# Z2PackDev/TBmodels

Measured on AMD Instinct MI355X. Metric: k-points/sec (H(k)+eig) at N_orb=64, N_R=4096, higher is better.
Workload: dtype f64; 1 GPU; cfg2: dense N_orb=64 N_R=4096, 100000 random k-points per GPU, eigenval (H(k)+eig); kpoints_per_gpu=100000, collective=none, rccl_ranks=0, eigensolver=auto

## Files before the change

### tbmodels_amd/csrc/tbk_eig_small.hip

```cpp

#include <cstdlib>
#include <type_traits>

#include "tbk_dpp.h"
#include "tbk_internal.h"

namespace {

typedef double d2 __attribute__((ext_vector_type(2)));

template <int CTRL>
__device__ __forceinline__ double dpp_mov(double v) {
    int lo = __double2loint(v), hi = __double2hiint(v);
    lo = __builtin_amdgcn_update_dpp(0, lo, CTRL, 0xf, 0xf, true);
    hi = __builtin_amdgcn_update_dpp(0, hi, CTRL, 0xf, 0xf, true);
    return __hiloint2double(hi, lo);
}

__device__ __forceinline__ double wave_sum(double v) {
    v += dpp_mov<0x128>(v);
    v += dpp_mov<0x124>(v);
    v += dpp_mov<0x122>(v);
    v += dpp_mov<0x121>(v);
    {
        const unsigned lo = (unsigned)__double2loint(v), hi = (unsigned)__double2hiint(v);
        const auto rl = __builtin_amdgcn_permlane16_swap(lo, lo, false, false);
        const auto rh = __builtin_amdgcn_permlane16_swap(hi, hi, false, false);
        v = __hiloint2double((int)rh[0], (int)rl[0]) + __hiloint2double((int)rh[1], (int)rl[1]);
    }
    {
        const unsigned lo = (unsigned)__double2loint(v), hi = (unsigned)__double2hiint(v);
        const auto rl = __builtin_amdgcn_permlane32_swap(lo, lo, false, false);
        const auto rh = __builtin_amdgcn_permlane32_swap(hi, hi, false, false);
        v = __hiloint2double((int)rh[0], (int)rl[0]) + __hiloint2double((int)rh[1], (int)rl[1]);
    }
    return v;
}

__device__ __forceinline__ void wg_sync() {
    asm volatile("s_waitcnt lgkmcnt(0)" ::: "memory");
    __syncthreads();
}

__device__ __forceinline__ double bcast(double v, int lane) { return __shfl(v, lane, 64); }
__device__ __forceinline__ double bcast_uniform(double v, int lane) {
    const int lo = __builtin_amdgcn_readlane(__double2loint(v), lane);
    const int hi = __builtin_amdgcn_readlane(__double2hiint(v), lane);
    return __hiloint2double(hi, lo);
}

__device__ __forceinline__ double fast_rcp(double x) {
    double r = __builtin_amdgcn_rcp(x);
    double e = fma(-x, r, 1.0);
    r = fma(r, e, r);
    e = fma(-x, r, 1.0);
    return fma(r, e, r);
}
__device__ __forceinline__ void fast_sqrt_rsqrt(double x, double& root, double& rroot) {
    double r = __builtin_amdgcn_rsq(x);
    double g = x * r, h = 0.5 * r;
    double e = fma(-h, g, 0.5);
    g = fma(g, e, g);
    h = fma(h, e, h);
    e = fma(-h, g, 0.5);
    g = fma(g, e, g);
    h = fma(h, e, h);
    const double d = fma(-g, g, x);
    root = fma(d, h, g);
    rroot = 2.0 * h;
    e = fma(-root, rroot, 1.0);
    rroot = fma(rroot, e, rroot);
}


__device__ __forceinline__ void wave_lds_fence() { asm volatile("s_waitcnt lgkmcnt(0)" ::: "memory"); }

template <int SEG>
__device__ __forceinline__ double seg_sum(double v) {
    if (SEG == 8) {
        v += dpp_mov<0x141>(v);
        v += dpp_mov<0xB1>(v);
        v += dpp_mov<0x4E>(v);
        return v;
    }
    v += dpp_mov<0x128>(v);
    v += dpp_mov<0x124>(v);
    v += dpp_mov<0x122>(v);
    v += dpp_mov<0x121>(v);
    if (SEG == 32) {
        const unsigned lo = (unsigned)__double2loint(v), hi = (unsigned)__double2hiint(v);
        const auto rl = __builtin_amdgcn_permlane16_swap(lo, lo, false, false);
        const auto rh = __builtin_amdgcn_permlane16_swap(hi, hi, false, false);
        v = __hiloint2double((int)rh[0], (int)rl[0]) + __hiloint2double((int)rh[1], (int)rl[1]);
    }
    return v;
}

template <int NRP>
__global__ void __launch_bounds__(64)
herm_tridiag_packed_kernel(const double* __restrict__ H, int n, int64_t nk, double* __restrict__ D,
                           double* __restrict__ E, int64_t h_stride, int ldd, int off) {
    constexpr int G = 64 / NRP;
    constexpr int CG = 4;
    constexpr int NGR = NRP / CG;
    __shared__ d2 sv[64];
    __shared__ d2 sw[64];
    const int lane = threadIdx.x;
    const int row = lane % NRP;
    const int base = lane - row;
    const int64_t mat = (int64_t)blockIdx.x * G + lane / NRP;
    const bool live = mat < nk;
    const int64_t mc = live ? mat : nk - 1;
    const double* Hm = H + (size_t)mc * h_stride;
    double* Dm = D + (size_t)mc * ldd + off;
    double* Em = E + (size_t)mc * ldd + off;

    double ar[NRP], ai[NRP];
    {
        constexpr int LB = NRP <= 16 ? NRP : 16;
        const int li = min(row, n - 1);
        static_for<0, NRP / LB>([&](auto hc) {
            constexpr int c0 = decltype(hc)::value * LB;
            d2 raw[LB];
#pragma unroll
            for (int u = 0; u < LB; ++u) {
                const int cc = min(c0 + u, n - 1);
                const int lo = min(li, cc), hi = max(li, cc);
                raw[u] = *reinterpret_cast<const d2*>(Hm + ((size_t)lo * n + hi) * 2);
            }
#pragma unroll
            for (int u = 0; u < LB; ++u) {
                const int c = c0 + u;
                const bool inside = row < n && c < n;
                ar[c] = inside ? raw[u][0] : 0.0;
                ai[c] = inside ? (c >= row ? raw[u][1] : -raw[u][1]) : 0.0;
            }
        });
    }
    double xr = ar[0], xi = ai[0];

    constexpr bool BC = NRP >= 16;
    constexpr int NB = NRP >= 16 ? NRP / 16 : 1;
    auto spread = [&](double x, double (&o)[NB]) {
        if constexpr (NRP == 32) {
            const unsigned xl = (unsigned)__double2loint(x), xh = (unsigned)__double2hiint(x);
            const auto rl = __builtin_amdgcn_permlane16_swap(xl, xl, false, false);
            const auto rh = __builtin_amdgcn_permlane16_swap(xh, xh, false, false);
            o[0] = __hiloint2double((int)rh[0], (int)rl[0]);
            o[NB - 1] = __hiloint2double((int)rh[1], (int)rl[1]);
        } else {
            o[0] = x;
        }
    };

    for (int j = 0; j < n - 1; ++j) {
        if (live && row == j) Dm[j] = xr;
        const double alr = __shfl(xr, base + j + 1, 64), ali = __shfl(xi, base + j + 1, 64);
        const bool below = (row > j + 1) && (row < n);
        const double sigma = seg_sum<NRP>(below ? (xr * xr + xi * xi) : 0.0);
        const bool done = (sigma == 0.0) && (ali == 0.0);
        double root, rroot;
        fast_sqrt_rsqrt(done ? 1.0 : alr * alr + ali * ali + sigma, root, rroot);
        const double beta = done ? alr : -copysign(root, alr);
        const double rbeta = done ? 0.0 : -copysign(rroot, alr);
        const double tr = (beta - alr) * rbeta, ti = -ali * rbeta;
        const double qr = alr - beta, qi = ali;
        const double qn = done ? 0.0 : fast_rcp(qr * qr + qi * qi);
        const double scr = qr * qn, sci = -qi * qn;
        if (live && row == 0) Em[j] = beta;

        double vr = 0.0, vi = 0.0;
        if (below) {
            vr = xr * scr - xi * sci;
            vi = xr * sci + xi * scr;
        } else if (row == j + 1) {
            vr = 1.0;
        }
        double vbr[NB], vbi[NB];
        if constexpr (BC) {
            spread(vr, vbr);
            spread(vi, vbi);
        } else {
            wave_lds_fence();
            sv[lane] = (d2){vr, vi};
            wave_lds_fence();
        }

        double pr = 0.0, pi = 0.0;
        {
            double par[CG], pai[CG];
#pragma unroll
            for (int cc = 0; cc < CG; ++cc) par[cc] = pai[cc] = 0.0;
            static_for<0, NGR>([&](auto grc) {
                constexpr int gr = decltype(grc)::value;
                if (gr * CG + CG - 1 > j) {
                    if constexpr (BC) {
                        static_for<0, CG>([&](auto ccc) {
                            constexpr int cc = decltype(ccc)::value, c = gr * CG + cc;
                            fmac_bc<c & 15>(par[cc], vbr[c >> 4], ar[c]);
                            fmac_bc<c & 15>(pai[cc], vbi[c >> 4], ar[c]);
                            fnmac_bc<c & 15>(par[cc], vbi[c >> 4], ai[c]);
                            fmac_bc<c & 15>(pai[cc], vbr[c >> 4], ai[c]);
                        });
                    } else {
                        d2 vb[CG];
#pragma unroll
                        for (int cc = 0; cc < CG; ++cc) vb[cc] = sv[base + gr * CG + cc];
#pragma unroll
                        for (int cc = 0; cc < CG; ++cc) {
                            par[cc] = fma(ar[gr * CG + cc], vb[cc][0], par[cc]);
                            pai[cc] = fma(ar[gr * CG + cc], vb[cc][1], pai[cc]);
                        }
#pragma unroll
                        for (int cc = 0; cc < CG; ++cc) {
                            par[cc] = fma(-ai[gr * CG + cc], vb[cc][1], par[cc]);
                            pai[cc] = fma(ai[gr * CG + cc], vb[cc][0], pai[cc]);
                        }
                    }
                }
            });
#pragma unroll
            for (int cc = 0; cc < CG; ++cc) {
                pr += par[cc];
                pi += pai[cc];
            }
        }
        if (!((row > j) && (row < n))) pr = pi = 0.0;
        const double rho = seg_sum<NRP>(pr * vr + pi * vi);
        const double a2 = -0.5 * (tr * tr + ti * ti) * rho;
        const double wr = fma(a2, vr, pr * tr - pi * ti);
        const double wi = fma(a2, vi, pr * ti + pi * tr);
        double wbr[NB], wbi[NB];
        if constexpr (BC) {
            spread(wr, wbr);
            spread(wi, wbi);
        } else {
            sw[lane] = (d2){wr, wi};
            wave_lds_fence();
        }

        double nxr = 0.0, nxi = 0.0;
        static_for<0, NGR>([&](auto grc) {
            constexpr int gr = decltype(grc)::value;
            if (gr * CG + CG - 1 > j) {
                if constexpr (BC) {
                    static_for<0, CG>([&](auto ccc) {
                        constexpr int cc = decltype(ccc)::value, c = gr * CG + cc;
                        double r = ar[c], mm = ai[c];
                        fnmac_bc<c & 15>(r, wbr[c >> 4], vr);
                        fnmac_bc<c & 15>(mm, wbr[c >> 4], vi);
                        fnmac_bc<c & 15>(r, wbi[c >> 4], vi);
                        fmac_bc<c & 15>(mm, wbi[c >> 4], vr);
                        fnmac_bc<c & 15>(r, vbr[c >> 4], wr);
                        fnmac_bc<c & 15>(mm, vbr[c >> 4], wi);
                        fnmac_bc<c & 15>(r, vbi[c >> 4], wi);
                        fmac_bc<c & 15>(mm, vbi[c >> 4], wr);
                        ar[c] = r;
                        ai[c] = mm;
                        if (c == j + 1) {
                            nxr = r;
                            nxi = mm;
                        }
                    });
                } else {
                    d2 vb[CG], wb[CG];
#pragma unroll
                    for (int cc = 0; cc < CG; ++cc) {
                        vb[cc] = sv[base + gr * CG + cc];
                        wb[cc] = sw[base + gr * CG + cc];
                    }
#pragma unroll
                    for (int cc = 0; cc < CG; ++cc) {
                        const int c = gr * CG + cc;
                        ar[c] = fma(-vr, wb[cc][0], ar[c]);
                        ai[c] = fma(-vi, wb[cc][0], ai[c]);
                        ar[c] = fma(-vi, wb[cc][1], ar[c]);
                        ai[c] = fma(vr, wb[cc][1], ai[c]);
                        ar[c] = fma(-wr, vb[cc][0], ar[c]);
                        ai[c] = fma(-wi, vb[cc][0], ai[c]);
                        ar[c] = fma(-wi, vb[cc][1], ar[c]);
                        ai[c] = fma(wr, vb[cc][1], ai[c]);
                        if (c == j + 1) {
                            nxr = ar[c];
                            nxi = ai[c];
                        }
                    }
                }
            }
        });
        xr = nxr;
        xi = nxi;
    }
    if (live && row == n - 1) Dm[n - 1] = xr;
    if (live && row == 0) Em[n - 1] = 0.0;
}

struct HhScalars {
    d2 tau;
    d2 flag;
};

template <int NR, int NW>
__global__ void __launch_bounds__(NW * 64, NW == 2 ? 2 : 4)
herm_tridiag4_kernel(double* H, int n, double* __restrict__ D, double* __restrict__ E, int n_steps, int64_t h_stride, int ldd,
                     int off) {
    const bool split = n_steps < n - 1;
    constexpr int NT = NR / NW;
    constexpr int NB = (NT + 15) / 16;
    constexpr int TB = 2;
    constexpr int HT = NT / NB;
    static_assert(NT % NB == 0, "columns per lane must split evenly over the register arrays");
    typedef double dcol __attribute__((ext_vector_type(HT)));
    __shared__ d2 sx[2][NR];
    __shared__ HhScalars ssc;
    __shared__ d2 sp[NW][NR];
    __shared__ d2 sw[NR];
    const int lane = threadIdx.x & 63;
    const int q = __builtin_amdgcn_readfirstlane(threadIdx.x >> 6);
    const size_t mat = blockIdx.x;
    double* Hm = H + mat * (size_t)h_stride;
    double* Dm = D + mat * (size_t)ldd + off;
    double* Em = E + mat * (size_t)ldd + off;

    dcol ar0, ai0, ar1, ai1;
    static_assert(NB <= 2, "at most 32 columns per lane");
    auto AR = [&](auto bc) -> dcol& { if constexpr (decltype(bc)::value == 0) return ar0; else return ar1; };
    auto AI = [&](auto bc) -> dcol& { if constexpr (decltype(bc)::value == 0) return ai0; else return ai1; };
#define TBK_AR(t) AR(std::integral_constant<int, (t) / HT>{})[(t) % HT]
#define TBK_AI(t) AI(std::integral_constant<int, (t) / HT>{})[(t) % HT]
    {
        constexpr int LB = NT <= 16 ? NT : NT / 2;
        const int li = min(lane, n - 1);
        static_for<0, NT / LB>([&](auto t0c) {
            constexpr int t0 = decltype(t0c)::value * LB;
            d2 raw[LB];
#pragma unroll
            for (int u = 0; u < LB; ++u) {
                const int c = min(NW * (t0 + u) + q, n - 1);
                const int lo = min(li, c), hi = max(li, c);
                raw[u] = *reinterpret_cast<const d2*>(Hm + ((size_t)lo * n + hi) * 2);
            }
            static_for<0, LB>([&](auto uc) {
                constexpr int u = decltype(uc)::value;
                const int c = NW * (t0 + u) + q;
                const bool inside = lane < n && c < n;
                TBK_AR(t0 + u) = inside ? raw[u][0] : 0.0;
                TBK_AI(t0 + u) = inside ? (c >= lane ? raw[u][1] : -raw[u][1]) : 0.0;
            });
        });
    }

    auto publish = [&](int jc) {
        const int tsel = jc / NW;
        double xr, xi;
        if (NB == 1 || tsel < HT) {
            xr = ar0[tsel % HT];
            xi = ai0[tsel % HT];
        } else {
            xr = ar1[tsel % HT];
            xi = ai1[tsel % HT];
        }
        if (lane == jc) Dm[jc] = xr;
        if (jc >= n - 1) {
            if (lane == 0) Em[n - 1] = 0.0;
            return;
        }
        const double alr = bcast_uniform(xr, jc + 1), ali = bcast_uniform(xi, jc + 1);
        const bool below = (lane > jc + 1) && (lane < n);
        const double sigma = wave_sum(below ? (xr * xr + xi * xi) : 0.0);
        HhScalars sc;
        double e_out;
        double vr = 0.0, vi = 0.0;
        if (sigma == 0.0 && ali == 0.0) {
            sc.tau = (d2){0.0, 0.0};
            sc.flag = (d2){1.0, 0.0};
            e_out = alr;
        } else {
            double root, rroot;
            fast_sqrt_rsqrt(alr * alr + ali * ali + sigma, root, rroot);
            const double beta = -copysign(root, alr);
            const double rbeta = -copysign(rroot, alr);
            const double qr = alr - beta, qi = ali;
            const double qn = fast_rcp(qr * qr + qi * qi);
            const double sr = qr * qn, si = -qi * qn;
            sc.tau = (d2){(beta - alr) * rbeta, -ali * rbeta};
            sc.flag = (d2){0.0, 0.0};
            e_out = beta;
            if (below) {
                vr = xr * sr - xi * si;
                vi = xr * si + xi * sr;
            } else if (lane == jc + 1) {
                vr = 1.0;
            }
        }
        if (lane < NR) sx[jc & 1][lane] = (d2){vr, vi};
        if (lane == 0) {
            ssc = sc;
            Em[jc] = e_out;
        }
    };
    if (q == 0) publish(0);
    int bc_slot[NB];
#pragma unroll
    for (int b = 0; b < NB; ++b) bc_slot[b] = min(NW * (16 * b + (lane & 15)) + q, NR - 1);

    for (int j = 0; j < n_steps; ++j) {
#ifdef TBK_ABLATE_CASCADE
        const unsigned pick = (blockIdx.x * 2654435761u) >> 20;
        if (NR == 64 && j >= 16 && (pick & 3) == 3) break;
        if (TBK_ABLATE_CASCADE == 2 && NR == 64 && j >= 8 && (pick & 7) == 6) break;
        if (TBK_ABLATE_CASCADE == 3 && NR == 64 && j >= 16) break;
        if (TBK_ABLATE_CASCADE == 4 && NR == 64 && j >= 1) break;
#endif
        wg_sync();
        const d2 vme = (lane < NR) ? sx[j & 1][lane] : (d2){0.0, 0.0};
        const HhScalars sc = ssc;
        const int jn = j + 1;
        const bool own_next = (jn & (NW - 1)) == q && !(split && jn == n_steps);
        if (__builtin_amdgcn_readfirstlane(__double2hiint(sc.flag[0])) != 0) {
            wg_sync();
            if (own_next) publish(jn);
            continue;
        }
        const double tr = sc.tau[0], ti = sc.tau[1];
        const double vr = vme[0], vi = vme[1];
        d2 vb[NB];
#pragma unroll
        for (int b = 0; b < NB; ++b) vb[b] = sx[j & 1][bc_slot[b]];

        double par[2] = {0.0, 0.0}, pai[2] = {0.0, 0.0};
        static_for<0, NT / TB>([&](auto tbc) {
            constexpr int tb = decltype(tbc)::value * TB;
            if (NW * (tb + TB) - 1 > j) {
                static_for<0, TB>([&](auto uc) {
                    constexpr int t = tb + decltype(uc)::value;
                    double a_re = TBK_AR(t), a_im = TBK_AI(t);
                    fmac_bc<t & 15>(par[t & 1], vb[t >> 4][0], a_re);
                    fmac_bc<t & 15>(pai[t & 1], vb[t >> 4][1], a_re);
                    fnmac_bc<t & 15>(par[t & 1], vb[t >> 4][1], a_im);
                    fmac_bc<t & 15>(pai[t & 1], vb[t >> 4][0], a_im);
                });
            }
        });
        if (lane < NR) sp[q][lane] = (d2){par[0] + par[1], pai[0] + pai[1]};
        wg_sync();
        double pr = 0.0, pi = 0.0;
        {
            d2 t[NW];
#pragma unroll
            for (int w = 0; w < NW; ++w) t[w] = sp[w][lane < NR ? lane : NR - 1];
#pragma unroll
            for (int w = 0; w < NW; ++w) {
                pr += t[w][0];
                pi += t[w][1];
            }
            if (!(lane > j && lane < n)) pr = pi = 0.0;
        }
        const double rho = wave_sum(pr * vr + pi * vi);
        const double a2 = -0.5 * (tr * tr + ti * ti) * rho;
        const double wr = fma(a2, vr, pr * tr - pi * ti);
        const double wi = fma(a2, vi, pr * ti + pi * tr);
        if (lane < NR) sw[lane] = (d2){wr, wi};
        wave_lds_fence();
        d2 wb[NB];
#pragma unroll
        for (int b = 0; b < NB; ++b) wb[b] = sw[bc_slot[b]];

        static_for<0, NT / TB>([&](auto tbc) {
            constexpr int tb = decltype(tbc)::value * TB;
            if (NW * (tb + TB) - 1 > j) {
                static_for<0, TB>([&](auto uc) {
                    constexpr int t = tb + decltype(uc)::value;
                    double r = TBK_AR(t), m = TBK_AI(t);
                    fnmac_bc<t & 15>(r, wb[t >> 4][0], vr);
                    fnmac_bc<t & 15>(m, wb[t >> 4][0], vi);
                    fnmac_bc<t & 15>(r, wb[t >> 4][1], vi);
                    fmac_bc<t & 15>(m, wb[t >> 4][1], vr);
                    fnmac_bc<t & 15>(r, vb[t >> 4][0], wr);
                    fnmac_bc<t & 15>(m, vb[t >> 4][0], wi);
                    fnmac_bc<t & 15>(r, vb[t >> 4][1], wi);
                    fmac_bc<t & 15>(m, vb[t >> 4][1], wr);
                    TBK_AR(t) = r;
                    TBK_AI(t) = m;
                });
            }
        });
        if (own_next) publish(jn);
    }
    if (split) {
        const int s0 = n_steps;
        static_for<0, NT>([&](auto tc) {
            constexpr int t = decltype(tc)::value;
            const int c = NW * t + q;
            if (c >= s0 && c < n && lane >= c && lane < n)
                *reinterpret_cast<d2*>(Hm + ((size_t)(c - s0) * 32 + (lane - s0)) * 2) = (d2){TBK_AR(t), -TBK_AI(t)};
        });
    }
#undef TBK_AR
#undef TBK_AI
}

constexpr int load_batch(int nt) {
    int best = 1;
    for (int d = 2; d <= 12; ++d)
        if (nt % d == 0) best = d;
    return best;
}

template <int NC, int NW>
__global__ void __launch_bounds__(NW * 128, 2)
herm_tridiag8_kernel(double* H, int n, double* __restrict__ D, double* __restrict__ E, int n_steps, int64_t h_stride, int ldd, int off) {
    constexpr int NR = 128;
    constexpr int NT = NC / NW;
    constexpr int NB = (NT + 15) / 16;
    constexpr int TB = 2;
    static_assert(NC % (NW * TB) == 0 && NB <= 3 && (NW == 2 || NW == 4), "column layout");
    __shared__ d2 sx[2][NR];
    __shared__ double ssig[2][2];
    __shared__ d2 sp[NW][NR];
    __shared__ double srho[2 * NW];
    const int lane = threadIdx.x & 63;
    const int wv = __builtin_amdgcn_readfirstlane(threadIdx.x >> 6);
    const int q = wv & (NW - 1), rh = wv / NW;
    const int row = rh * 64 + lane;
    const size_t mat = blockIdx.x;
    double* Hm = H + mat * (size_t)h_stride;
    double* Dm = D + mat * (size_t)ldd + off;
    double* Em = E + mat * (size_t)ldd + off;

    double ar[NT], ai[NT];
    {
        constexpr int LB = load_batch(NT);
        const int li = min(row, n - 1);
        static_for<0, NT / LB>([&](auto t0c) {
            constexpr int t0 = decltype(t0c)::value * LB;
            d2 raw[LB];
#pragma unroll
            for (int u = 0; u < LB; ++u) {
                const int c = min(NW * (t0 + u) + q, n - 1);
                const int lo = min(li, c), hi = max(li, c);
                raw[u] = *reinterpret_cast<const d2*>(Hm + ((size_t)lo * n + hi) * 2);
            }
            static_for<0, LB>([&](auto uc) {
                constexpr int u = decltype(uc)::value;
                const int c = NW * (t0 + u) + q;
                const bool inside = row < n && c < n;
                ar[t0 + u] = inside ? raw[u][0] : 0.0;
                ai[t0 + u] = inside ? (c >= row ? raw[u][1] : -raw[u][1]) : 0.0;
            });
        });
    }

    auto publish = [&](int jc, double xr, double xi) {
        if (row == jc) Dm[jc] = xr;
        const bool below = (row > jc + 1) && (row < n);
        const double part = wave_sum(below ? (xr * xr + xi * xi) : 0.0);
        sx[jc & 1][row] = (d2){xr, xi};
        if (lane == 0) ssig[jc & 1][rh] = part;
    };
    if (q == 0) publish(0, ar[0], ai[0]);
    int bc_col[NB];
#pragma unroll
    for (int b = 0; b < NB; ++b) bc_col[b] = NW * (16 * b + (lane & 15)) + q;

    for (int j = 0; j < n_steps; ++j) {
        wg_sync();
        const int jn = j + 1;
        const d2 xme = sx[j & 1][row];
        const d2 al = sx[j & 1][jn];
        const double sigma = ssig[j & 1][0] + ssig[j & 1][1];
        d2 xb[NB];
#pragma unroll
        for (int b = 0; b < NB; ++b) xb[b] = sx[j & 1][min(bc_col[b], NR - 1)];
        const bool own_next = (jn & (NW - 1)) == q && jn != n_steps;
        const int tn = own_next ? jn / NW : -1;
        const double alr = al[0], ali = al[1];
        const bool ident = sigma == 0.0 && ali == 0.0;
        double root, rroot;
        fast_sqrt_rsqrt(ident ? 1.0 : alr * alr + ali * ali + sigma, root, rroot);
        const double beta = -copysign(root, alr);
        const double rbeta = -copysign(rroot, alr);
        const double qr = alr - beta, qi = ali;
        const double qn = fast_rcp(ident ? 1.0 : qr * qr + qi * qi);
        const double sr = ident ? 0.0 : qr * qn, si = ident ? 0.0 : -qi * qn;
        double tr = ident ? 0.0 : (beta - alr) * rbeta, ti = ident ? 0.0 : -ali * rbeta;
        if (NT * 4 > 176) {
            tr = __hiloint2double(__builtin_amdgcn_readfirstlane(__double2hiint(tr)), __builtin_amdgcn_readfirstlane(__double2loint(tr)));
            ti = __hiloint2double(__builtin_amdgcn_readfirstlane(__double2hiint(ti)), __builtin_amdgcn_readfirstlane(__double2loint(ti)));
        }
        const double one = ident ? 0.0 : 1.0;
        if (wv == 0 && lane == 0) Em[j] = ident ? alr : beta;
        double vr = 0.0, vi = 0.0;
        if (row > jn && row < n) {
            vr = xme[0] * sr - xme[1] * si;
            vi = xme[0] * si + xme[1] * sr;
        } else if (row == jn) {
            vr = one;
        }
        d2 vb[NB];
#pragma unroll
        for (int b = 0; b < NB; ++b) {
            const int c = bc_col[b];
            vb[b] = (d2){0.0, 0.0};
            if (c > jn && c < n)
                vb[b] = (d2){xb[b][0] * sr - xb[b][1] * si, xb[b][0] * si + xb[b][1] * sr};
            else if (c == jn)
                vb[b] = (d2){one, 0.0};
        }

        double par[2] = {0.0, 0.0}, pai[2] = {0.0, 0.0};
        static_for<0, NT / TB>([&](auto tbc) {
            constexpr int tb = decltype(tbc)::value * TB;
            if (NW * (tb + TB) - 1 > j) {
                static_for<0, TB>([&](auto uc) {
                    constexpr int t = tb + decltype(uc)::value;
                    fmac_bc<t & 15>(par[t & 1], vb[t >> 4][0], ar[t]);
                    fmac_bc<t & 15>(pai[t & 1], vb[t >> 4][1], ar[t]);
                    fnmac_bc<t & 15>(par[t & 1], vb[t >> 4][1], ai[t]);
                    fmac_bc<t & 15>(pai[t & 1], vb[t >> 4][0], ai[t]);
                });
            }
        });
        {
            const double p_r = par[0] + par[1], p_i = pai[0] + pai[1];
            sp[q][row] = (d2){p_r, p_i};
            const double share = wave_sum((row > j && row < n) ? (p_r * vr + p_i * vi) : 0.0);
            if (lane == 0) srho[wv] = share;
        }
        wg_sync();
        double ur = 0.0, ui = 0.0, rho = 0.0;
        double ubr[NB], ubi[NB];
        {
            constexpr int B0 = (NT * 4 > 176 && NB > 1) ? 1 : NB;
            d2 t[NW], tb2[NB][NW];
            double rs[2 * NW];
#pragma unroll
            for (int w2 = 0; w2 < NW; ++w2) t[w2] = sp[w2][row];
#pragma unroll
            for (int b = 0; b < B0; ++b)
#pragma unroll
                for (int w2 = 0; w2 < NW; ++w2) tb2[b][w2] = sp[w2][min(bc_col[b], NR - 1)];
#pragma unroll
            for (int w2 = 0; w2 < 2 * NW; ++w2) rs[w2] = srho[w2];
#pragma unroll
            for (int w2 = 0; w2 < NW; ++w2) {
                ur += t[w2][0];
                ui += t[w2][1];
            }
#pragma unroll
            for (int w2 = 0; w2 < 2 * NW; ++w2) rho += rs[w2];
#pragma unroll
            for (int b = 0; b < NB; ++b) {
                if (b >= B0) {
                    asm volatile("" ::: "memory");
#pragma unroll
                    for (int w2 = 0; w2 < NW; ++w2) tb2[b][w2] = sp[w2][min(bc_col[b], NR - 1)];
                }
                ubr[b] = ubi[b] = 0.0;
#pragma unroll
                for (int w2 = 0; w2 < NW; ++w2) {
                    ubr[b] += tb2[b][w2][0];
                    ubi[b] += tb2[b][w2][1];
                }
                if (!(bc_col[b] > j && bc_col[b] < n)) ubr[b] = ubi[b] = 0.0;
            }
            if (!(row > j && row < n)) ur = ui = 0.0;
        }
        const double a2 = -0.5 * (tr * tr + ti * ti) * rho;
        const double wr = fma(a2, vr, ur * tr - ui * ti);
        const double wi = fma(a2, vi, ur * ti + ui * tr);
        d2 wb[NB];
#pragma unroll
        for (int b = 0; b < NB; ++b)
            wb[b] = (d2){fma(a2, vb[b][0], ubr[b] * tr - ubi[b] * ti), fma(a2, vb[b][1], ubr[b] * ti + ubi[b] * tr)};

        double nxr = 0.0, nxi = 0.0;
        static_for<0, NT / TB>([&](auto tbc) {
            constexpr int tb = decltype(tbc)::value * TB;
            if (NW * (tb + TB) - 1 > j) {
                static_for<0, TB>([&](auto uc) {
                    constexpr int t = tb + decltype(uc)::value;
                    double r = ar[t], m = ai[t];
                    fnmac_bc<t & 15>(r, wb[t >> 4][0], vr);
                    fnmac_bc<t & 15>(m, wb[t >> 4][0], vi);
                    fnmac_bc<t & 15>(r, wb[t >> 4][1], vi);
                    fmac_bc<t & 15>(m, wb[t >> 4][1], vr);
                    fnmac_bc<t & 15>(r, vb[t >> 4][0], wr);
                    fnmac_bc<t & 15>(m, vb[t >> 4][0], wi);
                    fnmac_bc<t & 15>(r, vb[t >> 4][1], wi);
                    fmac_bc<t & 15>(m, vb[t >> 4][1], wr);
                    ar[t] = r;
                    ai[t] = m;
                    if (t == tn) {
                        nxr = r;
                        nxi = m;
                        asm volatile("" : "+v"(nxr), "+v"(nxi));
                    }
                });
            }
        });
        if (own_next) publish(jn, nxr, nxi);
    }
    {
        const int s0 = n_steps;
        const int ldt = n - n_steps;
        static_for<0, NT>([&](auto tc) {
            constexpr int t = decltype(tc)::value;
            const int c = NW * t + q;
            if (c >= s0 && c < n && row >= c && row < n)
                *reinterpret_cast<d2*>(Hm + ((size_t)(c - s0) * ldt + (row - s0)) * 2) = (d2){ar[t], -ai[t]};
        });
    }
}


template <int QL_LD>
__global__ void __launch_bounds__(64)
tridiag_ql_kernel(const double* __restrict__ D, const double* __restrict__ E, int n, int64_t nk,
                  double* __restrict__ out, int* __restrict__ fail_count) {
    extern __shared__ __attribute__((aligned(16))) double ql_smem[];
    double* sd = ql_smem;
    double* se = ql_smem + (size_t)n * QL_LD;
    const int lane = threadIdx.x;
    const int64_t m0 = (int64_t)blockIdx.x * QL_LD;
    const int nmat = (int)min((int64_t)QL_LD, nk - m0);

    for (int idx = lane; idx < nmat * n; idx += 64) {
        const int mm = idx / n, c = idx % n;
        sd[c * QL_LD + mm] = D[m0 * n + idx];
        se[c * QL_LD + mm] = E[m0 * n + idx];
    }
    __syncthreads();

    if (lane < nmat) {
        double* d = sd + lane;
        double* e = se + lane;
        bool failed = false;
        bool finite = true;
        for (int i = 0; i < n; ++i) finite = finite && isfinite(d[i * QL_LD]) && isfinite(e[i * QL_LD]);
        if (!finite) {
            for (int i = 0; i < n; ++i) d[i * QL_LD] = __builtin_nan("");
            atomicAdd(fail_count + 1, 1);
        }
        const double EPS = 2.220446049250313e-16;
        int l = 0, m = 0, iter = 0;
        bool done = !finite;
        auto settle = [&]() {
            while (l < n - 1) {
                m = l;
                double ad = fabs(d[l * QL_LD]);
                for (; m < n - 1; ++m) {
                    const double ad1 = fabs(d[(m + 1) * QL_LD]);
                    if (fabs(e[m * QL_LD]) <= EPS * (ad + ad1)) break;
                    ad = ad1;
                }
                if (m != l) break;
                ++l;
            }
            if (l >= n - 1) done = true;
            iter = 0;
        };
        if (!done) settle();
        while (!done) {
            if (++iter > 60) {
                failed = true;
                break;
            }
            const double el = e[l * QL_LD];
            const double dl = d[l * QL_LD];
            double g = (d[(l + 1) * QL_LD] - dl) / (2.0 * el);
            double r = sqrt(fma(g, g, 1.0));
            g = d[m * QL_LD] - dl + el / (g + copysign(r, g));
            double s = 1.0, c = 1.0, p = 0.0;
            double d_up = d[m * QL_LD];
            double d_i = d[(m - 1) * QL_LD], e_i = e[(m - 1) * QL_LD];
            bool underflow = false;
            int m_next = m;
            double ad_prev = 0.0;
            for (int i = m - 1; i >= l; --i) {
                const int ip = (i > l) ? i - 1 : l;
                const double d_nx = d[ip * QL_LD], e_nx = e[ip * QL_LD];
                const double f = s * e_i;
                const double b = c * e_i;
                const double h2 = fma(f, f, g * g);
                if (h2 == 0.0) {
                    e[(i + 1) * QL_LD] = 0.0;
                    d[(i + 1) * QL_LD] = d_up - p;
                    e[m * QL_LD] = 0.0;
                    underflow = true;
                    break;
                }
                const double rinv = rsqrt(h2);
                const double e_new = h2 * rinv;
                e[(i + 1) * QL_LD] = e_new;
                s = f * rinv;
                c = g * rinv;
                const double gg = d_up - p;
                r = (d_i - gg) * s + 2.0 * c * b;
                p = s * r;
                const double d_new = gg + p;
                d[(i + 1) * QL_LD] = d_new;
                g = c * r - b;
                const double ad_cur = fabs(d_new);
                if (i + 1 < m && e_new <= EPS * (ad_cur + ad_prev)) m_next = i + 1;
                ad_prev = ad_cur;
                d_up = d_i;
                d_i = d_nx;
                e_i = e_nx;
            }
            if (underflow) {
                const int it = iter;
                settle();
                iter = it;
                continue;
            }
            const double dl_new = d_up - p;
            d[l * QL_LD] = dl_new;
            e[l * QL_LD] = g;
            e[m * QL_LD] = 0.0;
            m = m_next;
            if (fabs(g) <= EPS * (fabs(dl_new) + ad_prev)) {
                ++l;
                iter = 0;
                if (l >= m) settle();
            }
        }
        if (failed) atomicAdd(fail_count, 1);
        for (int a = 1; a < n && finite; ++a) {
            const double key = d[a * QL_LD];
            int b = a - 1;
            while (b >= 0 && d[b * QL_LD] > key) {
                d[(b + 1) * QL_LD] = d[b * QL_LD];
                --b;
            }
            d[(b + 1) * QL_LD] = key;
        }
    }
    __syncthreads();
    for (int idx = lane; idx < nmat * n; idx += 64) {
        const int mm = idx / n, c = idx % n;
        out[m0 * n + idx] = sd[c * QL_LD + mm];
    }
}

}

static int launch_tridiag_33_64(hipStream_t s, double* d_H, int n, int64_t nk, double* d_D, double* d_Eo, int64_t h_stride, int ldd, int off,
                                bool split_on) {
    const dim3 grid((unsigned)nk), block(64);
    const int n_steps = split_on ? n - 32 : n - 1;
#define TBK_T4(NRV, NWV) \
    hipLaunchKernelGGL((herm_tridiag4_kernel<NRV, NWV>), grid, dim3(NWV * 64), 0, s, d_H, n, d_D, d_Eo, n_steps, h_stride, ldd, off)
    if (n <= 40 && split_on)
        TBK_T4(40, 2);
    else if (n <= 48 && split_on)
        TBK_T4(48, 2);
    else if (n <= 48)
        TBK_T4(48, 4);
    else if (n <= 56 && split_on)
        TBK_T4(56, 2);
    else if (n <= 56)
        TBK_T4(56, 4);
    else if (split_on)
        TBK_T4(64, 2);
    else
        TBK_T4(64, 4);
#undef TBK_T4
    TBK_HIP(hipGetLastError());
    if (split_on) {
        hipLaunchKernelGGL(herm_tridiag_packed_kernel<32>, dim3((unsigned)((nk + 1) / 2)), block, 0, s, d_H, 32, nk, d_D, d_Eo,
                           h_stride, ldd, off + n - 32);
        TBK_HIP(hipGetLastError());
    }
    return TBK_OK;
}

int tbk_launch_tridiag_tail64(const tbk_eig_plan_t& plan, hipStream_t s, double* d_H, int64_t nk, double* d_D, double* d_E, int n_full) {
    return launch_tridiag_33_64(s, d_H, 64, nk, d_D, d_E, (int64_t)n_full * n_full * 2, n_full, n_full - 64, plan.split_on);
}

int tbk_launch_tridiag_reg128(const tbk_eig_plan_t& plan, hipStream_t s, double* d_H, int n, int64_t nk, double* d_D, double* d_E, int64_t h_stride, int ldd, int off) {
    const dim3 grid((unsigned)nk);
#define TBK_T8(NCV, NWV) \
    hipLaunchKernelGGL((herm_tridiag8_kernel<NCV, NWV>), grid, dim3(NWV * 128), 0, s, d_H, n, d_D, d_E, n - 64, h_stride, ldd, off)
    const bool nw2 = plan.reg128_nw2;
    if (n <= 80 && nw2)
        TBK_T8(80, 2);
    else if (n <= 80)
        TBK_T8(80, 4);
    else if (n <= 96 && nw2)
        TBK_T8(96, 2);
    else if (n <= 96)
        TBK_T8(96, 4);
    else if (n <= 112)
        TBK_T8(112, 4);
    else
        TBK_T8(128, 4);
#undef TBK_T8
    TBK_HIP(hipGetLastError());
    return TBK_OK;
}

int tbk_launch_tridiag(tbk_model* m, const tbk_eig_plan_t& plan, hipStream_t s, double* d_H, int64_t nk, double* d_de) {
    const int n = plan.n;
    if (nk == 0) return TBK_OK;
    double* d_D = d_de;
    double* d_Eo = d_de + (size_t)nk * n;
    StageTimer t(m, TBK_T_EIG, s);
    const dim3 block(64);
    const int64_t packed = (int64_t)n * n * 2;
    if (n > 32) return launch_tridiag_33_64(s, d_H, n, nk, d_D, d_Eo, packed, n, 0, plan.split_on);
    if (n <= 8)
        hipLaunchKernelGGL(herm_tridiag_packed_kernel<8>, dim3((unsigned)((nk + 7) / 8)), block, 0, s, d_H, n, nk, d_D, d_Eo, packed, n, 0);
    else if (n <= 16)
        hipLaunchKernelGGL(herm_tridiag_packed_kernel<16>, dim3((unsigned)((nk + 3) / 4)), block, 0, s, d_H, n, nk, d_D, d_Eo, packed, n, 0);
    else
        hipLaunchKernelGGL(herm_tridiag_packed_kernel<32>, dim3((unsigned)((nk + 1) / 2)), block, 0, s, d_H, n, nk, d_D, d_Eo, packed, n, 0);
    TBK_HIP(hipGetLastError());
    return TBK_OK;
}

int tbk_launch_ql(tbk_model* m, hipStream_t s, const double* d_de, int64_t nk, double* d_E, bool beside_ql) {
    const int n = m->n_orb;
    if (nk == 0) return TBK_OK;
    StageTimer t(m, TBK_T_QL, s);
#define TBK_QL_LAUNCH(MPB)                                                                                  \
    hipLaunchKernelGGL(tridiag_ql_kernel<MPB>, dim3((unsigned)((nk + MPB - 1) / MPB)), dim3(64),             \
                       (size_t)2 * n * MPB * sizeof(double), s, d_de, d_de + (size_t)nk * n, n, nk, d_E,     \
                       m->ws_flag.as<int>())
    if (n <= 64 && beside_ql && nk <= 8192) {
        TBK_QL_LAUNCH(32);
    } else if (n <= 64) {
        TBK_QL_LAUNCH(64);
    } else if (n <= 128) {
        TBK_QL_LAUNCH(32);
    } else if (n <= 256) {
        TBK_QL_LAUNCH(16);
    } else if (n <= 512) {
        TBK_QL_LAUNCH(8);
    } else {
        tbk_set_error("tridiagonal QL kernel handles n <= 512 (n = %d)", n);
        return TBK_ERR_ARGUMENT;
    }
#undef TBK_QL_LAUNCH
    TBK_HIP(hipGetLastError());
    return TBK_OK;
}
```

Baseline: 1.194 million k-points/s.

## Group Householder steps by column block to skip dead columns and publish early

Splits the tridiagonalization step loop into compile-time column groups. Within each group, only the still-active register columns are processed, and the rank-2 update of the next pivot column runs before the rest. That lets the next Householder vector be published (reflector computation and LDS write) before the remaining trailing-column updates, overlapping its serial reduction with bulk FMA work. It also replaces the runtime-indexed register selection in publish with a compile-time select and fuses several multiply-adds into fma. Code size and register pressure grow from the extra unrolling, and fma contraction slightly changes rounding.

```diff
diff --git a/tbmodels_amd/csrc/tbk_eig_small.hip b/tbmodels_amd/csrc/tbk_eig_small.hip
--- a/tbmodels_amd/csrc/tbk_eig_small.hip
+++ b/tbmodels_amd/csrc/tbk_eig_small.hip
@@ -350,16 +350,7 @@
         });
     }
 
-    auto publish = [&](int jc) {
-        const int tsel = jc / NW;
-        double xr, xi;
-        if (NB == 1 || tsel < HT) {
-            xr = ar0[tsel % HT];
-            xi = ai0[tsel % HT];
-        } else {
-            xr = ar1[tsel % HT];
-            xi = ai1[tsel % HT];
-        }
+    auto publish = [&](int jc, double xr, double xi) {
         if (lane == jc) Dm[jc] = xr;
         if (jc >= n - 1) {
             if (lane == 0) Em[n - 1] = 0.0;
@@ -367,7 +358,7 @@
         }
         const double alr = bcast_uniform(xr, jc + 1), ali = bcast_uniform(xi, jc + 1);
         const bool below = (lane > jc + 1) && (lane < n);
-        const double sigma = wave_sum(below ? (xr * xr + xi * xi) : 0.0);
+        const double sigma = wave_sum(below ? fma(xi, xi, xr * xr) : 0.0);
         HhScalars sc;
         double e_out;
         double vr = 0.0, vi = 0.0;
@@ -377,18 +368,18 @@
             e_out = alr;
         } else {
             double root, rroot;
-            fast_sqrt_rsqrt(alr * alr + ali * ali + sigma, root, rroot);
+            fast_sqrt_rsqrt(fma(alr, alr, ali * ali) + sigma, root, rroot);
             const double beta = -copysign(root, alr);
             const double rbeta = -copysign(rroot, alr);
             const double qr = alr - beta, qi = ali;
-            const double qn = fast_rcp(qr * qr + qi * qi);
+            const double qn = fast_rcp(fma(qr, qr, qi * qi));
             const double sr = qr * qn, si = -qi * qn;
             sc.tau = (d2){(beta - alr) * rbeta, -ali * rbeta};
             sc.flag = (d2){0.0, 0.0};
             e_out = beta;
             if (below) {
-                vr = xr * sr - xi * si;
-                vi = xr * si + xi * sr;
+                vr = fma(xr, sr, -(xi * si));
+                vi = fma(xr, si, xi * sr);
             } else if (lane == jc + 1) {
                 vr = 1.0;
             }
@@ -399,94 +390,124 @@
             Em[jc] = e_out;
         }
     };
-    if (q == 0) publish(0);
+    if (q == 0) publish(0, TBK_AR(0), TBK_AI(0));
     int bc_slot[NB];
 #pragma unroll
     for (int b = 0; b < NB; ++b) bc_slot[b] = min(NW * (16 * b + (lane & 15)) + q, NR - 1);
 
-    for (int j = 0; j < n_steps; ++j) {
+    int n_run = n_steps;
 #ifdef TBK_ABLATE_CASCADE
+    {
         const unsigned pick = (blockIdx.x * 2654435761u) >> 20;
-        if (NR == 64 && j >= 16 && (pick & 3) == 3) break;
-        if (TBK_ABLATE_CASCADE == 2 && NR == 64 && j >= 8 && (pick & 7) == 6) break;
-        if (TBK_ABLATE_CASCADE == 3 && NR == 64 && j >= 16) break;
-        if (TBK_ABLATE_CASCADE == 4 && NR == 64 && j >= 1) break;
+        if (NR == 64 && (pick & 3) == 3) n_run = min(n_run, 16);
+        if (TBK_ABLATE_CASCADE == 2 && NR == 64 && (pick & 7) == 6) n_run = min(n_run, 8);
+        if (TBK_ABLATE_CASCADE == 3 && NR == 64) n_run = min(n_run, 16);
+        if (TBK_ABLATE_CASCADE == 4 && NR == 64) n_run = min(n_run, 1);
+    }
 #endif
-        wg_sync();
-        const d2 vme = (lane < NR) ? sx[j & 1][lane] : (d2){0.0, 0.0};
-        const HhScalars sc = ssc;
-        const int jn = j + 1;
-        const bool own_next = (jn & (NW - 1)) == q && !(split && jn == n_steps);
-        if (__builtin_amdgcn_readfirstlane(__double2hiint(sc.flag[0])) != 0) {
+
+    constexpr int GB = 2;
+    constexpr int BS = NW * TB, GS = GB * BS;
+    constexpr int NG = (NR - 2) / GS + 1;
+    static_assert(NT % TB == 0 && (NG - 1) * GB < NT / TB, "column groups per lane split into skip blocks");
+    static_for<0, NG>([&](auto gc) {
+        constexpr int j0 = decltype(gc)::value * GS;
+        constexpr int T0 = decltype(gc)::value * GB * TB;
+        constexpr int T1 = T0 + GB * TB < NT ? T0 + GB * TB : NT;
+        constexpr int T2 = T1 + 1 < NT ? T1 + 1 : NT;
+        const int j1 = min(j0 + GS, n_run);
+        for (int j = j0; j < j1; ++j) {
             wg_sync();
-            if (own_next) publish(jn);
-            continue;
-        }
-        const double tr = sc.tau[0], ti = sc.tau[1];
-        const double vr = vme[0], vi = vme[1];
-        d2 vb[NB];
-#pragma unroll
-        for (int b = 0; b < NB; ++b) vb[b] = sx[j & 1][bc_slot[b]];
-
-        double par[2] = {0.0, 0.0}, pai[2] = {0.0, 0.0};
-        static_for<0, NT / TB>([&](auto tbc) {
-            constexpr int tb = decltype(tbc)::value * TB;
-            if (NW * (tb + TB) - 1 > j) {
-                static_for<0, TB>([&](auto uc) {
-                    constexpr int t = tb + decltype(uc)::value;
+            const d2 vme = (lane < NR) ? sx[j & 1][lane] : (d2){0.0, 0.0};
+            const HhScalars sc = ssc;
+            const int jn = j + 1;
+            const bool own_next = (jn & (NW - 1)) == q && !(split && jn == n_steps);
+            const bool flagged = __builtin_amdgcn_readfirstlane(__double2hiint(sc.flag[0])) != 0;
+            auto own_blocks = [&](auto&& col) {
+                static_for<0, GB>([&](auto ic) {
+                    constexpr int tb = T0 + decltype(ic)::value * TB;
+                    if constexpr (tb < NT) {
+                        if (NW * (tb + TB) - 1 > j) static_for<tb, tb + TB>(col);
+                    }
+                });
+            };
+            double vr = 0.0, vi = 0.0, wr = 0.0, wi = 0.0;
+            d2 vb[NB], wb[NB];
+#pragma unroll
+            for (int b = 0; b < NB; ++b) vb[b] = wb[b] = (d2){0.0, 0.0};
+            auto upd_col = [&](auto tc) {
+                constexpr int t = decltype(tc)::value;
+                double r = TBK_AR(t), m = TBK_AI(t);
+                fnmac_bc<t & 15>(r, wb[t >> 4][0], vr);
+                fnmac_bc<t & 15>(m, wb[t >> 4][0], vi);
+                fnmac_bc<t & 15>(r, wb[t >> 4][1], vi);
+                fmac_bc<t & 15>(m, wb[t >> 4][1], vr);
+                fnmac_bc<t & 15>(r, vb[t >> 4][0], wr);
+                fnmac_bc<t & 15>(m, vb[t >> 4][0], wi);
+                fnmac_bc<t & 15>(r, vb[t >> 4][1], wi);
+                fmac_bc<t & 15>(m, vb[t >> 4][1], wr);
+                TBK_AR(t) = r;
+                TBK_AI(t) = m;
+            };
+            if (flagged) {
+                wg_sync();
+            } else {
+                const double tr = sc.tau[0], ti = sc.tau[1];
+                vr = vme[0];
+                vi = vme[1];
+#pragma unroll
+                for (int b = 0; b < NB; ++b) vb[b] = sx[j & 1][bc_slot[b]];
+
+                double par[2] = {0.0, 0.0}, pai[2] = {0.0, 0.0};
+                auto mv_col = [&](auto tc) {
+                    constexpr int t = decltype(tc)::value;
                     double a_re = TBK_AR(t), a_im = TBK_AI(t);
                     fmac_bc<t & 15>(par[t & 1], vb[t >> 4][0], a_re);
                     fmac_bc<t & 15>(pai[t & 1], vb[t >> 4][1], a_re);
                     fnmac_bc<t & 15>(par[t & 1], vb[t >> 4][1], a_im);
                     fmac_bc<t & 15>(pai[t & 1], vb[t >> 4][0], a_im);
+                };
+                own_blocks(mv_col);
+                static_for<T1, NT>(mv_col);
+                if (lane < NR) sp[q][lane] = (d2){par[0] + par[1], pai[0] + pai[1]};
+                wg_sync();
+                double pr = 0.0, pi = 0.0;
+                {
+                    d2 t[NW];
+#pragma unroll
+                    for (int w = 0; w < NW; ++w) t[w] = sp[w][lane < NR ? lane : NR - 1];
+#pragma unroll
+                    for (int w = 0; w < NW; ++w) {
+                        pr += t[w][0];
+                        pi += t[w][1];
+                    }
+                    if (!(lane > j && lane < n)) pr = pi = 0.0;
+                }
+                const double rho = wave_sum(fma(vr, pr, vi * pi));
+                const double a2 = -0.5 * fma(tr, tr, ti * ti) * rho;
+                wr = fma(a2, vr, fma(tr, pr, -(ti * pi)));
+                wi = fma(a2, vi, fma(ti, pr, tr * pi));
+                if (lane < NR) sw[lane] = (d2){wr, wi};
+                wave_lds_fence();
+#pragma unroll
+                for (int b = 0; b < NB; ++b) wb[b] = sw[bc_slot[b]];
+                own_blocks(upd_col);
+                static_for<T1, T2>(upd_col);
+            }
+            if (own_next) {
+                double nxr = TBK_AR(T0), nxi = TBK_AI(T0);
+                static_for<T0 + 1, T2>([&](auto tc) {
+                    double cr = TBK_AR(decltype(tc)::value), ci = TBK_AI(decltype(tc)::value);
+                    asm("" : "+v"(cr), "+v"(ci));
+                    const bool here = jn / NW == decltype(tc)::value;
+                    nxr = here ? cr : nxr;
+                    nxi = here ? ci : nxi;
                 });
-            }
-        });
-        if (lane < NR) sp[q][lane] = (d2){par[0] + par[1], pai[0] + pai[1]};
-        wg_sync();
-        double pr = 0.0, pi = 0.0;
-        {
-            d2 t[NW];
-#pragma unroll
-            for (int w = 0; w < NW; ++w) t[w] = sp[w][lane < NR ? lane : NR - 1];
-#pragma unroll
-            for (int w = 0; w < NW; ++w) {
-                pr += t[w][0];
-                pi += t[w][1];
-            }
-            if (!(lane > j && lane < n)) pr = pi = 0.0;
-        }
-        const double rho = wave_sum(pr * vr + pi * vi);
-        const double a2 = -0.5 * (tr * tr + ti * ti) * rho;
-        const double wr = fma(a2, vr, pr * tr - pi * ti);
-        const double wi = fma(a2, vi, pr * ti + pi * tr);
-        if (lane < NR) sw[lane] = (d2){wr, wi};
-        wave_lds_fence();
-        d2 wb[NB];
-#pragma unroll
-        for (int b = 0; b < NB; ++b) wb[b] = sw[bc_slot[b]];
-
-        static_for<0, NT / TB>([&](auto tbc) {
-            constexpr int tb = decltype(tbc)::value * TB;
-            if (NW * (tb + TB) - 1 > j) {
-                static_for<0, TB>([&](auto uc) {
-                    constexpr int t = tb + decltype(uc)::value;
-                    double r = TBK_AR(t), m = TBK_AI(t);
-                    fnmac_bc<t & 15>(r, wb[t >> 4][0], vr);
-                    fnmac_bc<t & 15>(m, wb[t >> 4][0], vi);
-                    fnmac_bc<t & 15>(r, wb[t >> 4][1], vi);
-                    fmac_bc<t & 15>(m, wb[t >> 4][1], vr);
-                    fnmac_bc<t & 15>(r, vb[t >> 4][0], wr);
-                    fnmac_bc<t & 15>(m, vb[t >> 4][0], wi);
-                    fnmac_bc<t & 15>(r, vb[t >> 4][1], wi);
-                    fmac_bc<t & 15>(m, vb[t >> 4][1], wr);
-                    TBK_AR(t) = r;
-                    TBK_AI(t) = m;
-                });
-            }
-        });
-        if (own_next) publish(jn);
-    }
+                publish(jn, nxr, nxi);
+            }
+            if (!flagged) static_for<T2, NT>(upd_col);
+        }
+    });
     if (split) {
         const int s0 = n_steps;
         static_for<0, NT>([&](auto tc) {
```

Result: no change. 1.192 million k-points/s (-0.1%).
